# luisdamiano/sparseRGPs

Hardware: AMD Instinct MI355X
Metric: sparse-GP objective+gradient evals/sec at n=1e6, m=1024, d=8 (higher is better)
Workload: dtype f64; 1 GPU; C3: Titsias VI ELBO + gradient, n=1000000, m=1024, d=8, ard, P=10, knots fixed; n=1000000, m=1024, d=8, kernel=ard, parallelism=single

## Files before the change

### sparsergps_amd/csrc/k_mfma.hip

```cpp
#include <algorithm>
#include <vector>

#include "sgp_internal.h"
#include "sgp_probe.h"
#include "sgp_syrk_plan.h"

namespace {

constexpr int T128 = 128;
constexpr int BK = 16;
constexpr int SB = 144;
constexpr int SA = 17;
constexpr int SYRK_RGRP = 16;

__device__ __forceinline__ double wave_sum(double v) {
#pragma unroll
  for (int o = 32; o > 0; o >>= 1) v += __shfl_xor(v, o, 64);
  return v;
}

__device__ __forceinline__ int64_t xcd_remap(int64_t orig, int64_t nwg) {
  return sgp_plan::xcd_remap(orig, nwg);
}

__device__ __forceinline__ void load8(const double* __restrict__ g, double2 (&v)[4]) {
  const double2* p = reinterpret_cast<const double2*>(g);
#pragma unroll
  for (int q = 0; q < 4; ++q) v[q] = p[q];
}
__device__ __forceinline__ void store8(double* s, const double2 (&v)[4]) {
  double2* p = reinterpret_cast<double2*>(s);
#pragma unroll
  for (int q = 0; q < 4; ++q) p[q] = v[q];
}

__device__ __forceinline__ void syrk_group(int64_t gi, int nb, int wv, int& ta, int& tb, int& rs,
                                           int& cs, int& rp, int& cp) {
  const int64_t noff = (int64_t)nb * (nb - 1) / 2;
  if (gi < noff) {
    int a = (int)((sqrtf(8.0f * (float)gi + 1.0f) + 1.0f) * 0.5f);
    while ((int64_t)a * (a - 1) / 2 > gi) --a;
    while ((int64_t)(a + 1) * a / 2 <= gi) ++a;
    const int b = (int)(gi - (int64_t)a * (a - 1) / 2);
    ta = a; tb = b;
    const int wr = wv >> 1, wc = wv & 1;
    rs = wr; cs = 2 + wc;
    rp = 2 * a + wr; cp = 2 * b + wc;
    return;
  }
  const int g = (int)(gi - noff), G = (3 * nb + 3) / 4;
  const int te = G + g / 3, kind = g % 3;
  ta = g;
  tb = (te < nb) ? te : g;
  if (wv == 0) { rs = 0; cs = 0; rp = 2 * g; cp = 2 * g; }
  else if (wv == 1) { rs = 1; cs = 0; rp = 2 * g + 1; cp = 2 * g; }
  else if (wv == 2) { rs = 1; cs = 1; rp = 2 * g + 1; cp = 2 * g + 1; }
  else if (te < nb) {
    if (kind == 0) { rs = 2; cs = 2; rp = 2 * te; cp = 2 * te; }
    else if (kind == 1) { rs = 3; cs = 2; rp = 2 * te + 1; cp = 2 * te; }
    else { rs = 3; cs = 3; rp = 2 * te + 1; cp = 2 * te + 1; }
  } else {
    rs = cs = rp = cp = -1;
  }
}

struct SyrkTMap {
  signed char e[128];
  int S;
};

template <bool SPREAD = false, int PAT = 0, int NVMEM = 8, int NMFMA = 64>
__device__ __forceinline__ void mfma_interleave() {
#pragma unroll
  for (int i = 0; i < NMFMA; ++i) {
    __builtin_amdgcn_sched_group_barrier(0x008, 1, 0);
    if (i >= SGP_IL_VMEM0 && i < SGP_IL_VMEM0 + NVMEM)
      __builtin_amdgcn_sched_group_barrier(0x020, 1, 0);
    if (SPREAD ? (i & 1) == 0 : i < 32)
      __builtin_amdgcn_sched_group_barrier(0x100, 1, 0);
    constexpr int w0 = PAT == 2 ? NMFMA - 8 : PAT == 3 ? NMFMA / 2 : NMFMA - 16;
    if (PAT != 4 && i >= w0 && i < w0 + 8)
      __builtin_amdgcn_sched_group_barrier(0x200, 1, 0);
  }
}

template <int V, int WMODE, int TMODE, bool COMPACT = false>
__device__ __forceinline__ void syrk_dt_body(const double* __restrict__ K, int64_t mp,
                                             const double* __restrict__ w,
                                             const double* __restrict__ r,
                                             const double* __restrict__ tv, int t, int64_t rbeg,
                                             int nsteps, double (*Ka)[BK * SB], double (*ws)[BK],
                                             double (*rw)[BK], double& tacc, double& rrp,
                                             double* __restrict__ out) {
  constexpr int R0 = V, R1 = 7 - V, N0 = R0 + 1, N1 = R1 + 1;
  constexpr bool WITH_T = TMODE != 0;
  const int tid = threadIdx.x, lane = tid & 63;
  d4 acc0[N0], acc1[N1];
#pragma unroll
  for (int c = 0; c < N0; ++c) acc0[c] = d4{0.0, 0.0, 0.0, 0.0};
#pragma unroll
  for (int c = 0; c < N1; ++c) acc1[c] = d4{0.0, 0.0, 0.0, 0.0};
  const int lrow = tid >> 4, lc = tid & 15;
  const double2* gA = reinterpret_cast<const double2*>(K + (rbeg + lrow) * mp + t * (int64_t)T128) + lc;
  const int64_t gstep = BK * mp / 2;
  double2 v[4];
  double vw = 1.0, vsa = 1.0, vrr = 0.0, vr = 0.0;
  double t4[4] = {0.0, 0.0, 0.0, 0.0};
  const int tcol = tid & (T128 - 1), trow = tid >> 7;
#define SDT_GLOAD(step)                                                         \
  {                                                                             \
    const int64_t o_ = (int64_t)(step) * gstep;                                 \
    const int64_t rr_ = rbeg + (int64_t)(step) * BK + (tid & (BK - 1));        \
    _Pragma("unroll") for (int q = 0; q < 4; ++q) v[q] = gA[o_ + 16 * q];       \
    if constexpr (WMODE == 1) vw = w[rr_];                                      \
    if constexpr (WMODE == 2) vsa = w[rbeg + (int64_t)(step) * BK + lrow];      \
    if constexpr (WITH_T) {                                                     \
      vrr = r[rr_];                                                             \
      if constexpr (TMODE == 2) vr = tv[rr_];                                   \
    }                                                                           \
  }
#define SDT_SSTORE(buf, fold)                                                   \
  {                                                                             \
    double2* p_ = reinterpret_cast<double2*>(&Ka[buf][lrow * SB]) + lc;         \
    _Pragma("unroll") for (int q = 0; q < 4; ++q) {                             \
      double2 x_ = v[q];                                                        \
      if constexpr (WMODE == 2) { x_.x *= vsa; x_.y *= vsa; }                   \
      p_[16 * q] = x_;                                                          \
    }                                                                           \
    if constexpr (WMODE == 1) ws[buf][tid & (BK - 1)] = vw;                     \
    if constexpr (WITH_T) {                                                     \
      const double rw_ = TMODE == 2 ? vr : vw * vrr;                            \
      rw[buf][tid & (BK - 1)] = rw_;                                            \
      rrp = fma(rw_ * (fold), vrr, rrp);                                        \
    }                                                                           \
  }
  if (nsteps > 0) {
    SDT_GLOAD(0);
    SDT_SSTORE(0, 1.0);
  }
  __syncthreads();
  for (int step = 0; step < nsteps; ++step) {
    const int cur = step & 1;
    const bool more = step + 1 < nsteps;
    SDT_GLOAD(more ? step + 1 : step);
    const double* Kc = Ka[cur];
#pragma unroll
    for (int kk = 0; kk < 4; ++kk) {
      const int krow = kk * 4 + (lane >> 4);
      const double* row = Kc + krow * SB + (lane & 15);
      double a0 = row[R0 * 16], a1 = row[R1 * 16];
      if constexpr (WMODE == 1) {
        const double wk = ws[cur][krow];
        a0 *= wk;
        a1 *= wk;
      }
#pragma unroll
      for (int c = 0; c < N1; ++c) {
        const double b = row[c * 16];
        if (c < N0) acc0[c] = __builtin_amdgcn_mfma_f64_16x16x4f64(a0, b, acc0[c], 0, 0, 0);
        acc1[c] = __builtin_amdgcn_mfma_f64_16x16x4f64(a1, b, acc1[c], 0, 0, 0);
      }
    }
    if constexpr (WITH_T) {
#pragma unroll
      for (int k = 0; k < BK / 2; ++k) {
        const int q = trow + 2 * k;
        t4[k & 3] = fma(rw[cur][q], Kc[q * SB + tcol], t4[k & 3]);
      }
    }
    SDT_SSTORE(cur ^ 1, more ? 1.0 : 0.0);
    if constexpr (SGP_SDT_IL && WMODE != 1) mfma_interleave<false, 2, 4, 36>();
    __syncthreads();
  }
#undef SDT_GLOAD
#undef SDT_SSTORE
  tacc = (t4[0] + t4[1]) + (t4[2] + t4[3]);
#pragma unroll
  for (int c = 0; c < N1; ++c)
#pragma unroll
    for (int hh = 0; hh < 2; ++hh) {
      if (hh == 0 && c >= N0) continue;
      const int R = hh == 0 ? R0 : R1;
      const d4& a = hh == 0 ? acc0[c] : acc1[c];
      const int rp = 2 * t + R / 4, cp = 2 * t + c / 4;
      double* blk = out + (COMPACT ? (int64_t)(R / 4 + c / 4)
                                   : (int64_t)(rp * (rp + 1) / 2 + cp)) * 4096;
#pragma unroll
      for (int q = 0; q < 4; ++q)
        blk[((R % 4) * 16 + (lane >> 4) + 4 * q) * 64 + (c % 4) * 16 + (lane & 15)] = a[q];
    }
}

template <int WMODE, int TMODE>
__device__ __forceinline__ void syrk_dtile(const double* __restrict__ K, int64_t n_pad,
                                           int64_t mp, const double* __restrict__ w,
                                           const double* __restrict__ r,
                                           const double* __restrict__ tv, int t, int nb,
                                           int64_t sd, int64_t chunk, double (*Ka)[BK * SB],
                                           double (*ws)[BK], double (*rw)[BK],
                                           double* __restrict__ out,
                                           double* __restrict__ slab_t,
                                           double* __restrict__ slab_rr) {
  const int64_t rbeg = sd * chunk;
  int64_t rend = rbeg + chunk;
  if (rend > n_pad) rend = n_pad;
  const int nsteps = rend > rbeg ? (int)((rend - rbeg) / BK) : 0;
  double tacc = 0.0, rrp = 0.0;
  switch (threadIdx.x >> 6) {
    case 0: syrk_dt_body<0, WMODE, TMODE>(K, mp, w, r, tv, t, rbeg, nsteps, Ka, ws, rw, tacc, rrp, out); break;
    case 1: syrk_dt_body<1, WMODE, TMODE>(K, mp, w, r, tv, t, rbeg, nsteps, Ka, ws, rw, tacc, rrp, out); break;
    case 2: syrk_dt_body<2, WMODE, TMODE>(K, mp, w, r, tv, t, rbeg, nsteps, Ka, ws, rw, tacc, rrp, out); break;
    default: syrk_dt_body<3, WMODE, TMODE>(K, mp, w, r, tv, t, rbeg, nsteps, Ka, ws, rw, tacc, rrp, out); break;
  }
  if constexpr (TMODE != 0) {
    const int tid = threadIdx.x;
    double* tsh = &Ka[0][0];
    tsh[tid] = tacc;
    __syncthreads();
    if (tid < T128) slab_t[(sd * nb + t) * T128 + tid] = tsh[tid] + tsh[tid + T128];
    if (t == 0 && tid < 64) {
      double v = tid < BK ? rrp : 0.0;
#pragma unroll
      for (int o = 32; o > 0; o >>= 1) v += __shfl_xor(v, o, 64);
      if (tid == 0) slab_rr[sd] = v;
    }
  }
}

template <int TMODE, int WMODE, int TR = 2>
__global__ void __launch_bounds__(256, 2)
k_syrk_blk(const double* __restrict__ K, int64_t n_pad, int64_t mp, const double* __restrict__ w,
           const double* __restrict__ r, const double* __restrict__ tv,
           int64_t chunk, int ngroups, int nb, double* __restrict__ slab,
           double* __restrict__ slab_t, double* __restrict__ slab_rr, SyrkTMap tm,
           int64_t nwg_blk, int64_t chunk_d, double* __restrict__ slab_d) {
  __shared__ __attribute__((aligned(16))) double Ka[2][BK * SB];
  __shared__ __attribute__((aligned(16))) double Kb[2][BK * SB];
  __shared__ double ws[2][BK];
  __shared__ double rw[2][BK];

  if constexpr (TMODE == 0 || WMODE == 3) {
    if ((int64_t)blockIdx.x >= nwg_blk) {
      const int64_t loc = (int64_t)blockIdx.x - nwg_blk;
      const int t = (int)(loc % nb);
      const int64_t sd = loc / nb;
      syrk_dtile<WMODE == 3 ? 1 : WMODE, TMODE>(
          K, n_pad, mp, w, r, tv, t, nb, sd, chunk_d, Ka, ws, rw,
          slab_d + sd * ((int64_t)(2 * nb) * (2 * nb + 1) / 2) * 4096, slab_t, slab_rr);
      return;
    }
  }
  const int64_t nwg = nwg_blk;
  const int64_t wgid = xcd_remap(blockIdx.x, nwg);
  const int split = (int)(wgid / ngroups);
  const int64_t gi = wgid % ngroups;
// ... 87 lines not shown
  }
  __syncthreads();
  for (int step = 0; step < nsteps; ++step) {
    const int cur = step & 1;
    const bool more = step + 1 < nsteps;
    SYRKB_GLOAD(more ? step + 1 : step);
    if constexpr (WITH_T) __builtin_amdgcn_sched_barrier(0);
    const double* As = (ra ? Kb[cur] : Ka[cur]) + ro;
    const double* Bs = (ca_ ? Kb[cur] : Ka[cur]) + co;
    {
#pragma unroll
      for (int kk = 0; kk < 4; ++kk) {
        const int krow = kk * 4 + (lane >> 4);
        double af[4], bf[4];
#pragma unroll
        for (int f = 0; f < 4; ++f) {
          af[f] = As[krow * SB + f * 16 + (lane & 15)];
          bf[f] = Bs[krow * SB + f * 16 + (lane & 15)];
        }
        if constexpr (WMODE == 1) {
          const double wk = ws[cur][krow];
#pragma unroll
          for (int f = 0; f < 4; ++f) af[f] *= wk;
        }
#pragma unroll
        for (int fm = 0; fm < 4; ++fm)
#pragma unroll
          for (int fn = 0; fn < 4; ++fn)
            acc[fm][fn] = __builtin_amdgcn_mfma_f64_16x16x4f64(af[fm], bf[fn], acc[fm][fn], 0, 0, 0);
      }
    }
    SYRKB_SSTORE(cur ^ 1, more ? 1.0 : 0.0);
    mfma_interleave<false, SGP_SYRK_IL_PAT, WITH_T ? 0 : 8>();
    if constexpr (WITH_T) {
      const double* img = (t_inb ? Kb[cur] : Ka[cur]) + tcol;
      double a_[TR], b_[TR];
#pragma unroll
      for (int k = 0; k < TR; ++k) {
        const int q = trg + k * (BK / TR);
        a_[k] = rw[cur][q];
        b_[k] = img[q * SB];
      }
#pragma unroll
      for (int k = 0; k < TR; ++k) tacc4[k & 3] = fma(a_[k], b_[k], tacc4[k & 3]);
    }
    __syncthreads();
  }
#undef SYRKB_GLOAD
#undef SYRKB_SSTORE

  if constexpr (WITH_T) {
    __syncthreads();
    double* tsh = &Ka[0][0];
    if (t_on) tsh[tid] = (tacc4[0] + tacc4[1]) + (tacc4[2] + tacc4[3]);
    __syncthreads();
    if (t_on && tid < tW) {
      double v = 0.0;
      for (int g = 0; g < tng; ++g) v += tsh[tid + g * tW];
      slab_t[((int64_t)split * nb + tpan) * T128 + tcol] = v;
    }
  }
  if (dg == 0 && with_t && wv == 0) {
    double v = t_rr ? rrp : 0.0;
#pragma unroll
    for (int o = 32; o > 0; o >>= 1) v += __shfl_xor(v, o, 64);
    if (tid == 0) slab_rr[split] = v;
  }
  if (!active) return;
  const int64_t bid = (int64_t)rp * (rp + 1) / 2 + cp;
  const int64_t nblk = (int64_t)(2 * nb) * (2 * nb + 1) / 2;
  double* out = slab + ((int64_t)split * nblk + bid) * 4096;
#pragma unroll
  for (int fm = 0; fm < 4; ++fm)
#pragma unroll
    for (int fn = 0; fn < 4; ++fn)
#pragma unroll
      for (int q = 0; q < 4; ++q) {
        const int row = fm * 16 + (lane >> 4) + 4 * q;
        const int col = fn * 16 + (lane & 15);
        out[row * 64 + col] = acc[fm][fn][q];
      }
}

__device__ __forceinline__ void syrk_off_seg(const double* __restrict__ K, int64_t mp, int ta,
                                             int tb, int64_t rbeg, int nsteps,
                                             double (*Ka)[BK * SB], double (*Kb)[BK * SB],
                                             double* __restrict__ out) {
  const int tid = threadIdx.x, lane = tid & 63, wv = tid >> 6;
  d4 acc[4][4];
#pragma unroll
  for (int a = 0; a < 4; ++a)
#pragma unroll
    for (int b = 0; b < 4; ++b) acc[a][b] = d4{0.0, 0.0, 0.0, 0.0};
  const int lrow = tid >> 4, lc = tid & 15;
  const double2* gA = reinterpret_cast<const double2*>(K + (rbeg + lrow) * mp + ta * (int64_t)T128) + lc;
  const double2* gB = reinterpret_cast<const double2*>(K + (rbeg + lrow) * mp + tb * (int64_t)T128) + lc;
  const int64_t gstep = BK * mp / 2;
  double2 va0, va1, va2, va3, vb0, vb1, vb2, vb3;
  const int ro = (wv >> 1) * 64, co = (wv & 1) * 64;
#define SYRKO_GLOAD(step)                                                       \
  {                                                                             \
    const int64_t o_ = (int64_t)(step) * gstep;                                 \
    va0 = gA[o_]; va1 = gA[o_ + 16]; va2 = gA[o_ + 32]; va3 = gA[o_ + 48];      \
    vb0 = gB[o_]; vb1 = gB[o_ + 16]; vb2 = gB[o_ + 32]; vb3 = gB[o_ + 48];      \
  }
#define SYRKO_SSTORE(buf)                                                       \
  {                                                                             \
    double2* pa_ = reinterpret_cast<double2*>(&Ka[buf][lrow * SB]) + lc;        \
    double2* pb_ = reinterpret_cast<double2*>(&Kb[buf][lrow * SB]) + lc;        \
    pa_[0] = va0; pa_[16] = va1; pa_[32] = va2; pa_[48] = va3;                  \
    pb_[0] = vb0; pb_[16] = vb1; pb_[32] = vb2; pb_[48] = vb3;                  \
  }
  SYRKO_GLOAD(0);
  SYRKO_SSTORE(0);
  __syncthreads();
  for (int step = 0; step < nsteps; ++step) {
    const int cur = step & 1;
    const bool more = step + 1 < nsteps;
    SYRKO_GLOAD(more ? step + 1 : step);
    const double* As = Ka[cur] + ro;
    const double* Bs = Kb[cur] + co;
#pragma unroll
    for (int kk = 0; kk < 4; ++kk) {
      const int krow = kk * 4 + (lane >> 4);
      double af[4], bf[4];
#pragma unroll
      for (int f = 0; f < 4; ++f) {
        af[f] = As[krow * SB + f * 16 + (lane & 15)];
        bf[f] = Bs[krow * SB + f * 16 + (lane & 15)];
      }
#pragma unroll
      for (int fm = 0; fm < 4; ++fm)
#pragma unroll
        for (int fn = 0; fn < 4; ++fn)
          acc[fm][fn] = __builtin_amdgcn_mfma_f64_16x16x4f64(af[fm], bf[fn], acc[fm][fn], 0, 0, 0);
    }
    SYRKO_SSTORE(cur ^ 1);
    mfma_interleave<false, SGP_SYRK_IL_PAT, 8>();
    __syncthreads();
  }
#undef SYRKO_GLOAD
#undef SYRKO_SSTORE
  double* blk = out + (int64_t)wv * 4096;
#pragma unroll
  for (int fm = 0; fm < 4; ++fm)
#pragma unroll
    for (int fn = 0; fn < 4; ++fn)
#pragma unroll
      for (int q = 0; q < 4; ++q) {
        const int row = fm * 16 + (lane >> 4) + 4 * q;
        const int col = fn * 16 + (lane & 15);
        blk[row * 64 + col] = acc[fm][fn][q];
      }
}

__device__ __forceinline__ void syrk_diag_seg(const double* __restrict__ K, int64_t mp, int t,
                                              int64_t rbeg, int nsteps, double (*Ka)[BK * SB],
                                              double* __restrict__ out) {
  double tacc = 0.0, rrp = 0.0;
  switch (threadIdx.x >> 6) {
    case 0: syrk_dt_body<0, 0, 0, true>(K, mp, nullptr, nullptr, nullptr, t, rbeg, nsteps, Ka, nullptr, nullptr, tacc, rrp, out); break;
    case 1: syrk_dt_body<1, 0, 0, true>(K, mp, nullptr, nullptr, nullptr, t, rbeg, nsteps, Ka, nullptr, nullptr, tacc, rrp, out); break;
    case 2: syrk_dt_body<2, 0, 0, true>(K, mp, nullptr, nullptr, nullptr, t, rbeg, nsteps, Ka, nullptr, nullptr, tacc, rrp, out); break;
    default: syrk_dt_body<3, 0, 0, true>(K, mp, nullptr, nullptr, nullptr, t, rbeg, nsteps, Ka, nullptr, nullptr, tacc, rrp, out); break;
  }
}

__global__ void __launch_bounds__(256, 2)
k_syrk_bal(const double* __restrict__ K, int64_t mp, sgp_plan::SyrkBalPlan p,
           double* __restrict__ slab_o, double* __restrict__ slab_d) {
  __shared__ __attribute__((aligned(16))) double Ka[2][BK * SB];
  __shared__ __attribute__((aligned(16))) double Kb[2][BK * SB];
  const int wg = (int)blockIdx.x < p.M ? (int)xcd_remap(blockIdx.x, p.M) : (int)blockIdx.x;
  sgp_plan::SyrkSeg s0, s1;
  sgp_plan::syrk_bp_segments(p, wg, s0, s1);
  if (s0.kind == sgp_plan::SEG_OFF) {
    int ta, tb;
    sgp_plan::syrk_off_panels(s0.id, ta, tb);
    syrk_off_seg(K, mp, ta, tb, s0.step0 * BK, s0.nsteps, Ka, Kb,
                 slab_o + ((int64_t)s0.slab * p.noff + s0.id) * 4 * 4096);
  } else if (s0.kind == sgp_plan::SEG_DIAG) {
    syrk_diag_seg(K, mp, s0.id, s0.step0 * BK, s0.nsteps, Ka, slab_d + (int64_t)s0.slab * 3 * 4096);
  }
  if (s1.kind == sgp_plan::SEG_DIAG)
    syrk_diag_seg(K, mp, s1.id, s1.step0 * BK, s1.nsteps, Ka, slab_d + (int64_t)s1.slab * 3 * 4096);
}

__global__ void __launch_bounds__(256)
k_syrk_reduce_bal(const double* __restrict__ slab_o, const double* __restrict__ slab_d,
                  sgp_plan::SyrkBalPlan p, int64_t mp, double* __restrict__ red,
                  const double* __restrict__ rr_src, double* __restrict__ rr_dst, int packed) {
  const int64_t bid = blockIdx.y;
  const int e = blockIdx.x * 256 + threadIdx.x;
  if (rr_src && bid == 0 && e < 8) rr_dst[e] = e == 0 ? *rr_src : 0.0;
  int rp = (int)((sqrtf(8.0f * (float)bid + 1.0f) - 1.0f) * 0.5f);
  while ((int64_t)(rp + 1) * (rp + 2) / 2 <= bid) ++rp;
  while ((int64_t)rp * (rp + 1) / 2 > bid) --rp;
  const int cp = (int)(bid - (int64_t)rp * (rp + 1) / 2);
  const bool upper = rp == cp && (e / 64) / 16 < (e % 64) / 16;
  if (upper && !packed) return;
  if (!packed && rp == cp && (e / 64) < (e % 64)) return;
  const double* src;
  int64_t stride;
  int cnt;
  if (rp / 2 == cp / 2) {
    const int t = rp / 2;
    src = slab_d + ((int64_t)p.sfirst[t] * 3 + (rp & 1) + (cp & 1)) * 4096 + e;
    stride = 3 * 4096;
    cnt = p.sfirst[t + 1] - p.sfirst[t];
  } else {
    const int a = rp / 2, b = cp / 2, gi = a * (a - 1) / 2 + b;
    src = slab_o + ((int64_t)gi * 4 + (rp & 1) * 2 + (cp & 1)) * 4096 + e;
    stride = (int64_t)p.noff * 4 * 4096;
    cnt = p.B;
  }
  double v = 0.0;
  if (!upper)
    for (int s0 = 0; s0 < cnt; s0 += 16) {
      double a[16];
#pragma unroll
      for (int q = 0; q < 16; ++q) a[q] = s0 + q < cnt ? src[(int64_t)(s0 + q) * stride] : 0.0;
#pragma unroll
// ... 291 lines not shown
    double2* pb_ = reinterpret_cast<double2*>(&Kb[buf][lrow * SB]) + lc;        \
    pa_[0] = va0; pa_[16] = va1; pa_[32] = va2; pa_[48] = va3;                  \
    pb_[0] = vb0; pb_[16] = vb1; pb_[32] = vb2; pb_[48] = vb3;                  \
  }
  if (nsteps > 0) {
    TN_GLOAD(0);
    TN_SSTORE(0);
  }
  __syncthreads();
  for (int step = 0; step < nsteps; ++step) {
    const int cur = step & 1;
    if (step + 1 < nsteps) TN_GLOAD(step + 1);
    const double* As = Ka[cur];
    const double* Bs = Kb[cur];
#pragma unroll
    for (int kk = 0; kk < 4; ++kk) {
      const int krow = kk * 4 + (lane >> 4);
      double af[4], bf[4];
#pragma unroll
      for (int f = 0; f < 4; ++f) {
        af[f] = As[krow * SB + wr * 64 + f * 16 + (lane & 15)];
        bf[f] = Bs[krow * SB + wc * 64 + f * 16 + (lane & 15)];
      }
#pragma unroll
      for (int fm = 0; fm < 4; ++fm)
#pragma unroll
        for (int fn = 0; fn < 4; ++fn)
          acc[fm][fn] = __builtin_amdgcn_mfma_f64_16x16x4f64(af[fm], bf[fn], acc[fm][fn], 0, 0, 0);
    }
    if (step + 1 < nsteps) TN_SSTORE(cur ^ 1);
    __syncthreads();
  }
#undef TN_GLOAD
#undef TN_SSTORE
  double* out = slab + ((int64_t)split * ntile + tile) * (T128 * T128);
#pragma unroll
  for (int fm = 0; fm < 4; ++fm)
#pragma unroll
    for (int fn = 0; fn < 4; ++fn)
#pragma unroll
      for (int q = 0; q < 4; ++q) {
        const int row = wr * 64 + fm * 16 + (lane >> 4) + 4 * q;
        const int col = wc * 64 + fn * 16 + (lane & 15);
        out[row * T128 + col] = acc[fm][fn][q];
      }
}

__global__ void __launch_bounds__(256)
k_gemm_tn_reduce(const double* __restrict__ slab, int splits, int nta, int ntb,
                 double* __restrict__ C) {
  const int tile = blockIdx.y;
  const int e = blockIdx.x * 256 + threadIdx.x;
  const int ntile = nta * ntb;
  double s = 0.0;
  for (int sp = 0; sp < splits; ++sp) s += slab[((int64_t)sp * ntile + tile) * (T128 * T128) + e];
  const int ta = tile / ntb, tb = tile % ntb;
  const int64_t a = (int64_t)ta * T128 + e / T128, b = (int64_t)tb * T128 + e % T128;
  C[a * (int64_t)ntb * T128 + b] = s;
}

__global__ void __launch_bounds__(256)
k_syrk_reduce_t(const double* __restrict__ slab_t, const double* __restrict__ slab_rr,
                int splits, int nb, int64_t mp, double* __restrict__ red) {
  const int64_t a = (int64_t)blockIdx.x * 256 + threadIdx.x;
  if (a < mp) {
    const int ta = (int)(a / T128), col = (int)(a % T128);
    double s = 0.0;
    for (int sp = 0; sp < splits; ++sp) s += slab_t[((int64_t)sp * nb + ta) * T128 + col];
    red[mp * mp + a] = s;
  }
  if (blockIdx.x == 0 && threadIdx.x == 0) {
    double s = 0.0;
    for (int sp = 0; sp < splits; ++sp) s += slab_rr[sp];
    red[mp * mp + mp] = s;
  }
}

enum { EPI_GRAD = 0, EPI_ROWQUAD = 1 };

constexpr int CON_A_SZ = T128 * SA;
constexpr int CON_B_SZ = BK * SB;
constexpr int CON_LDS = 2 * (CON_A_SZ + CON_B_SZ);

enum { CON_FULL = 0, CON_TAIL = 1, CON_HEAD = 2 };
constexpr int64_t CON_SK_SLOT = 65 * 256;
struct ConSK {
  double* ws = nullptr;
  int dp = -1;
  unsigned* flags = nullptr;
  unsigned epoch = 0;
  int64_t slot = 0;
  int* status = nullptr;
};

__device__ __forceinline__ unsigned con_ldu_sc1(const unsigned* p) {
  return __hip_atomic_load(p, __ATOMIC_RELAXED, __HIP_MEMORY_SCOPE_AGENT);
}

template <int DT, int EPI, bool V2, bool KNOT, bool FROM_T, bool KU, bool T2, int SKM,
          bool VIF = false>
__device__ __forceinline__ void con_tile(
    const KernParams& kp, const double* __restrict__ K, const double* __restrict__ M,
    const double* __restrict__ X, int64_t ldx, int64_t n, int64_t n_pad,
    const double* __restrict__ U, int64_t ldu, int64_t m, int64_t mp, const ConArgs& ca,
    double* __restrict__ slab, int nrec, double* __restrict__ rowq, int64_t ti, int64_t tj,
    int64_t wgid, int kb, int ke, double* lds, double (*red)[SGP_MAXD + 5], double (*s_uk)[BK],
    const ConSK& sk, int part, int tid_in) {
  const double* __restrict__ r = ca.r;
  const double* __restrict__ uvec = ca.uvec;
  const double* __restrict__ cdiag = ca.cdiag;
  constexpr int A_SZ = CON_A_SZ, B_SZ = CON_B_SZ;
  const int64_t ntj = mp / T128;
  const int64_t nwg = (n_pad / T128) * ntj;
  const int64_t i0 = ti * T128, j0 = tj * T128;

  const int tid = tid_in, lane = tid & 63, wv = tid >> 6;
  const int wr = wv >> 1, wc = wv & 1;
  const bool with_u = KU && (uvec != nullptr) && (ca.alpha_in == nullptr);
  constexpr bool with_v = V2;
  constexpr bool NOCS = VIF && !KNOT;

  d4 acc[4][4];
#pragma unroll
  for (int a = 0; a < 4; ++a)
#pragma unroll
    for (int b = 0; b < 4; ++b) acc[a][b] = d4{0.0, 0.0, 0.0, 0.0};

  const int arow = tid >> 1, acol = (tid & 1) * 8;
  const double2* gA = reinterpret_cast<const double2*>(K + (i0 + arow) * mp + acol);
  const int bk = tid >> 4, bc = tid & 15;
  const double2* gB = reinterpret_cast<const double2*>(M + (int64_t)bk * mp + j0) + bc;
  const int64_t bstep = BK * mp / 2;
  double2 va0, va1, va2, va3, vb0, vb1, vb2, vb3;
  double ku = 0.0, vuk = 0.0;
  const double* __restrict__ uk_src = with_u ? uvec : M;

#define CON_GLOAD(step)                                                          \
  {                                                                              \
    const int64_t oa_ = (int64_t)(step) * (BK / 2), ob_ = (int64_t)(step) * bstep; \
    va0 = gA[oa_]; va1 = gA[oa_ + 1]; va2 = gA[oa_ + 2]; va3 = gA[oa_ + 3];      \
    vb0 = gB[ob_]; vb1 = gB[ob_ + 16]; vb2 = gB[ob_ + 32]; vb3 = gB[ob_ + 48];   \
    if constexpr (KU) vuk = uk_src[(int64_t)(step) * BK + (tid & (BK - 1))];     \
  }
#define CON_SSTORE(buf)                                                          \
  {                                                                              \
    double* As_ = lds + (buf) * (A_SZ + B_SZ);                                   \
    double* pa_ = &As_[arow * SA + acol];                                        \
    double2* pb_ = reinterpret_cast<double2*>(&As_[A_SZ + bk * SB]) + bc;        \
    pa_[0] = va0.x; pa_[1] = va0.y; pa_[2] = va1.x; pa_[3] = va1.y;              \
    pa_[4] = va2.x; pa_[5] = va2.y; pa_[6] = va3.x; pa_[7] = va3.y;              \
    pb_[0] = vb0; pb_[16] = vb1; pb_[32] = vb2; pb_[48] = vb3;                   \
    if constexpr (KU) s_uk[buf][tid & (BK - 1)] = vuk;    \
  }
#define CON_KU(buf)                                                              \
  {                                                                              \
    const double* u_ = &s_uk[buf][acol];                                         \
    ku = fma(va0.x, u_[0], ku); ku = fma(va0.y, u_[1], ku);                      \
    ku = fma(va1.x, u_[2], ku); ku = fma(va1.y, u_[3], ku);                      \
    ku = fma(va2.x, u_[4], ku); ku = fma(va2.y, u_[5], ku);                      \
    ku = fma(va3.x, u_[6], ku); ku = fma(va3.y, u_[7], ku);                      \
  }

  SGP_PROBE_CON_STAMP(0);
  if constexpr (FROM_T) {
#pragma unroll
    for (int fm = 0; fm < 4; ++fm)
#pragma unroll
      for (int fn = 0; fn < 4; ++fn)
#pragma unroll
        for (int q = 0; q < 4; ++q)
          acc[fm][fn][q] = ca.tin[(i0 + wr * 64 + fm * 16 + (lane >> 4) + 4 * q) * mp + j0 +
                                  wc * 64 + fn * 16 + (lane & 15)];
  } else {
  CON_GLOAD(kb);
  CON_SSTORE(0);
  __syncthreads();
  for (int step = kb; step < ke; ++step) {
    const int cur = (step - kb) & 1;
    if constexpr (KU) CON_KU(cur);
    CON_GLOAD(step + 1 < ke ? step + 1 : step);
    const double* As = lds + cur * (A_SZ + B_SZ);
    const double* Bs = As + A_SZ;
#pragma unroll
    for (int kk = 0; kk < 4; ++kk) {
      const int kx = kk * 4 + (lane >> 4);
      double af[4], bf[4];
#pragma unroll
      for (int f = 0; f < 4; ++f) {
        af[f] = As[(wr * 64 + f * 16 + (lane & 15)) * SA + kx];
        bf[f] = Bs[kx * SB + wc * 64 + f * 16 + (lane & 15)];
      }
#pragma unroll
      for (int fm = 0; fm < 4; ++fm)
#pragma unroll
        for (int fn = 0; fn < 4; ++fn)
          acc[fm][fn] = __builtin_amdgcn_mfma_f64_16x16x4f64(af[fm], bf[fn], acc[fm][fn], 0, 0, 0);
    }
    CON_SSTORE(cur ^ 1);
    mfma_interleave<SGP_CON_IL_SPREAD, SGP_CON_IL_PAT>();
    __syncthreads();
  }
  }
#undef CON_GLOAD
#undef CON_SSTORE
#undef CON_KU

  if constexpr (SKM == CON_TAIL) {
    double* w = sk.ws + sk.slot * CON_SK_SLOT;
#pragma unroll
    for (int fm = 0; fm < 4; ++fm)
#pragma unroll
      for (int fn = 0; fn < 4; ++fn)
#pragma unroll
        for (int q = 0; q < 4; ++q)
          __hip_atomic_store(&w[((fm * 4 + fn) * 4 + q) * 256 + tid], acc[fm][fn][q],
                             __ATOMIC_RELAXED, __HIP_MEMORY_SCOPE_AGENT);
    __hip_atomic_store(&w[64 * 256 + tid], ku, __ATOMIC_RELAXED, __HIP_MEMORY_SCOPE_AGENT);
    asm volatile("s_waitcnt vmcnt(0)" ::: "memory");
    __syncthreads();
    if (tid == 0)
      __hip_atomic_store(&sk.flags[sk.slot], sk.epoch, __ATOMIC_RELAXED, __HIP_MEMORY_SCOPE_AGENT);
    return;
  }
  if (SKM == CON_HEAD && part == CON_HEAD) {
    if (tid == 0) {
      unsigned it = 0;
      while (con_ldu_sc1(&sk.flags[sk.slot]) != sk.epoch) {
        if (++it >= (1u << 22)) {
          atomicExch(sk.status, -1);
          break;
        }
        __builtin_amdgcn_s_sleep(1);
      }
    }
    __syncthreads();
    const double* w = sk.ws + sk.slot * CON_SK_SLOT;
#pragma unroll
    for (int fm = 0; fm < 4; ++fm) {
      double t[4][4];
#pragma unroll
      for (int fn = 0; fn < 4; ++fn)
#pragma unroll
        for (int q = 0; q < 4; ++q)
          t[fn][q] = __hip_atomic_load(&w[((fm * 4 + fn) * 4 + q) * 256 + tid], __ATOMIC_RELAXED,
                                       __HIP_MEMORY_SCOPE_AGENT);
#pragma unroll
      for (int fn = 0; fn < 4; ++fn)
#pragma unroll
        for (int q = 0; q < 4; ++q) acc[fm][fn][q] += t[fn][q];
      __builtin_amdgcn_sched_barrier(0);
    }
    ku += __hip_atomic_load(&w[64 * 256 + tid], __ATOMIC_RELAXED, __HIP_MEMORY_SCOPE_AGENT);
  }

  SGP_PROBE_CON_STAMP(1);
// ... 236 lines not shown
        const bool cok = 8 * ch + cc < d;
        double E = 0.0;
#pragma unroll
        for (int fn = 0; fn < 4; ++fn) {
          if constexpr (NOCS) {
#pragma unroll
            for (int q = 0; q < 4; ++q) {
              const int jl = wc * 64 + fn * 16 + (lane >> 4) + 4 * q;
              const double u = cok ? s_us[jl * sus + cc] : 0.0;
              const double pv = P[fn][q];
              E += (cp >= 8) ? pv : -2.0 * (u * pv);
            }
          } else {
          double C = Cc[fn];
          C += __shfl_xor(C, 16, 64);
          C += __shfl_xor(C, 32, 64);
          if (ch == 0 && (lane >> 4) == 0) e_sig += C;
#pragma unroll
          for (int q = 0; q < 4; ++q) {
            const int jl = wc * 64 + fn * 16 + (lane >> 4) + 4 * q;
            const double Cq = __shfl(C, (lane >> 4) + 4 * q, 64);
            const double u = cok ? s_us[jl * sus + cc] : 0.0;
            const double pv = P[fn][q];
            E += (cp >= 8) ? pv : u * fma(u, Cq, -2.0 * pv);
            if constexpr (KNOT) {
              if (cp < 8) s_kn[(wr * T128 + jl) * 8 + cc] = pv - u * Cq;
            }
          }
          }
        }
        E += __shfl_xor(E, 8, 64);
        E += __shfl_xor(E, 16, 64);
        E += __shfl_xor(E, 32, 64);
        if (ard) {
          if (lane < 8 && 8 * ch + lane < d) red[wv][1 + 8 * ch + lane] = E;
        } else {
          double t = E;
          t += __shfl_xor(t, 1, 64);
          t += __shfl_xor(t, 2, 64);
          t += __shfl_xor(t, 4, 64);
          e_sq += t;
        }
        if constexpr (KNOT) {
          __syncthreads();
          for (int e = tid; e < T128 * 8; e += 256) {
            const int col = e >> 3, c = e & 7, cg = 8 * ch + c;
            if (cg < d)
              ca.knot_slab[(ti * mp + j0 + col) * d + cg] =
                  s_kn[col * 8 + c] + s_kn[(T128 + col) * 8 + c];
          }
        }
      }
#undef CON_XSTAGE
    }

    SGP_PROBE_CON_STAMP(6);
    double v = 0.0;
    if constexpr (!NOCS) v = wave_sum(e_sig);
    if (lane == 0) red[wv][0] = v;
    if (!ard && lane == 0) red[wv][1] = e_sq * rl2s;
    v = 0.0;
    if constexpr (!VIF) v = wave_sum(a2);
    if (lane == 0) {
      red[wv][1 + L] = 0.0;
      red[wv][2 + L] = 0.0;
      red[wv][3 + L] = 0.0;
      red[wv][4 + L] = v;
    }
    __syncthreads();
    if (tid < nrec)
      slab[tid * nwg + wgid] = red[0][tid] + red[1][tid] + red[2][tid] + red[3][tid];
    SGP_PROBE_CON_STAMP(2);
  }
  if constexpr (SGP_CON_EPI_PRIO > 0) __builtin_amdgcn_s_setprio(0);
}

template <int DT, int EPI, bool V2 = false, bool KNOT = false, bool FROM_T = false, bool KU = true,
          bool T2 = false, bool VIF = false>
__global__ void __launch_bounds__(256, 2)
k_contract(KernParams kp, const double* __restrict__ K, const double* __restrict__ M,
           const double* __restrict__ X, int64_t ldx, int64_t n, int64_t n_pad,
           const double* __restrict__ U, int64_t ldu, int64_t m, int64_t mp, ConArgs ca,
           double* __restrict__ slab, int nrec, double* __restrict__ rowq) {
  __shared__ __attribute__((aligned(16))) double lds[CON_LDS];
  __shared__ double red[4][SGP_MAXD + 5];
  __shared__ double s_uk[2][BK];
  const int64_t ntj = mp / T128;
  const int64_t nwg = (n_pad / T128) * ntj;
  const int64_t wgid = xcd_remap(blockIdx.x, nwg);
  con_tile<DT, EPI, V2, KNOT, FROM_T, KU, T2, 0, VIF>(
      kp, K, M, X, ldx, n, n_pad, U, ldu, m, mp, ca, slab, nrec, rowq, wgid / ntj, wgid % ntj,
      wgid, 0, (int)(mp / BK), lds, red, s_uk, ConSK{}, CON_FULL, (int)threadIdx.x);
}

template <int DT, bool KNOT, bool VIF = false>
__global__ void __launch_bounds__(256, 2)
k_contract_sk(KernParams kp, const double* __restrict__ K, const double* __restrict__ M,
              const double* __restrict__ X, int64_t ldx, int64_t n, int64_t n_pad,
              const double* __restrict__ U, int64_t ldu, int64_t m, int64_t mp, ConArgs ca,
              double* __restrict__ slab, int nrec, ConSK sk) {
  __shared__ __attribute__((aligned(16))) double lds[CON_LDS];
  __shared__ double red[4][SGP_MAXD + 5];
  __shared__ double s_uk[2][BK];
  const int64_t ntj = mp / T128;
  const int64_t ntiles = (n_pad / T128) * ntj;
  const int S = (int)(mp / BK);
  const int64_t G = gridDim.x, v = xcd_remap(blockIdx.x, G);
  const int64_t dp_rounds = (sk.dp >= 0 && sk.dp < ntiles / G) ? sk.dp : ntiles / G - 1;
  const int64_t t0 = dp_rounds * G;
  const int64_t Usk = (ntiles - t0) * S;
  const int64_t u1 = Usk * (v + 1) / G;
  int64_t u = Usk * v / G;
  if (u % S != 0) {
    const int64_t tile = t0 + u / S;
    const int kb = (int)(u % S);
    ConSK p = sk;
    p.slot = v;
    con_tile<DT, EPI_GRAD, false, KNOT, false, !VIF, false, CON_TAIL, VIF>(
        kp, K, M, X, ldx, n, n_pad, U, ldu, m, mp, ca, slab, nrec, nullptr, tile / ntj,
        tile % ntj, tile, kb, S, lds, red, s_uk, p, CON_TAIL, (int)threadIdx.x);
    u += S - kb;
    __syncthreads();
  }
  int64_t r = 0;
  for (;;) {
    int64_t tile;
    int ke;
    if (r < dp_rounds) {
      tile = r * G + v;
      ke = S;
      ++r;
    } else if (u < u1) {
      tile = t0 + u / S;
      ke = (int)((u1 - u) < (int64_t)S ? (u1 - u) : S);
      u += ke;
    } else {
      break;
    }
    ConSK p = sk;
    p.slot = v + 1;
    int tid;
    asm volatile("v_mov_b32 %0, %1" : "=v"(tid) : "v"((int)threadIdx.x));
    con_tile<DT, EPI_GRAD, false, KNOT, false, !VIF, false, CON_HEAD, VIF>(
        kp, K, M, X, ldx, n, n_pad, U, ldu, m, mp, ca, slab, nrec, nullptr, tile / ntj,
        tile % ntj, tile, 0, ke, lds, red, s_uk, p, ke < S ? CON_HEAD : CON_FULL, tid);
    __syncthreads();
  }
}

__global__ void __launch_bounds__(256)
k_knot_reduce1(const double* __restrict__ slab, int64_t ntiles, int64_t ncol,
               double* __restrict__ part) {
  const int64_t col = (int64_t)blockIdx.x * 256 + threadIdx.x;
  const int64_t r = blockIdx.y, G = gridDim.y;
  if (col >= ncol) return;
  double s0 = 0.0, s1 = 0.0, s2 = 0.0, s3 = 0.0;
  int64_t t = r;
  for (; t + 3 * G < ntiles; t += 4 * G) {
    s0 += slab[t * ncol + col];
    s1 += slab[(t + G) * ncol + col];
    s2 += slab[(t + 2 * G) * ncol + col];
    s3 += slab[(t + 3 * G) * ncol + col];
  }
  for (; t < ntiles; t += G) s0 += slab[t * ncol + col];
  part[r * ncol + col] = (s0 + s1) + (s2 + s3);
}

// ... 852 lines not shown
```

### sparsergps_amd/csrc/sgp_probe.h

```cpp
#pragma once

#if (defined(SGP_CON_TRACE) || defined(SGP_CON_NO_EPILOGUE) || defined(SGP_GJ_TRACE) ||       \
     defined(SGP_IL_VMEM0) || defined(SGP_CON_IL_PAT) || defined(SGP_SYRK_IL_PAT) ||          \
     defined(SGP_CON_IL_SPREAD) || defined(SGP_CON_SHMEM) ||                                  \
     defined(SGP_SYRK_BAL) || defined(SGP_SYRK_WB) || defined(SGP_SYRK_WB_SLOTS) ||           \
     defined(SGP_SDT_IL) || defined(SGP_S256_IL) ||                  \
     defined(SGP_SDT_W) || defined(SGP_SDT_WW) || defined(SGP_SDT_WT) ||                      \
     defined(SGP_SYRK_W3) || defined(SGP_CON_ROWQ_KU) ||                                      \
     defined(SGP_LAP_RS_CFG) || defined(SGP_GJ_MM_UNROLL) || defined(SGP_VI_BUILD_NO_T) ||        \
     defined(SGP_GJ_STEPS) || defined(SGP_GJ_GMAX) || defined(SGP_CHAIN_US_STEP) ||         \
     defined(SGP_CHAIN_US_FIX) || defined(SGP_HOST_PROBE) || defined(SGP_BUILD_OCC_T2) ||      \
     defined(SGP_CON_EPI_PRIO) || defined(SGP_CON_PROBE_NO_EPI_MFMA) ||                       \
     defined(SGP_CON_PROBE_NO_KDMA)) &&      \
    !defined(SGP_PROBE_BUILD)
#error "timing probes and experiment knobs are for variant builds only (SGP_PROBE_BUILD)"
#endif

#ifndef SGP_CON_EPI_PRIO
#define SGP_CON_EPI_PRIO 0
#endif
#ifndef SGP_BUILD_OCC_T2
#define SGP_BUILD_OCC_T2 4
#endif
#ifndef SGP_IL_VMEM0
#define SGP_IL_VMEM0 0
#endif
#ifndef SGP_CON_IL_PAT
#define SGP_CON_IL_PAT 2
#endif
#ifndef SGP_SYRK_IL_PAT
#define SGP_SYRK_IL_PAT 0
#endif
#ifndef SGP_CON_IL_SPREAD
#define SGP_CON_IL_SPREAD false
#endif
#ifndef SGP_CON_SHMEM
#define SGP_CON_SHMEM 0
#endif
#ifndef SGP_SYRK_BAL
#define SGP_SYRK_BAL 1
#endif
#ifndef SGP_SYRK_WB
#define SGP_SYRK_WB 1
#endif
#ifndef SGP_SYRK_WB_SLOTS
#define SGP_SYRK_WB_SLOTS 512
#endif
#ifndef SGP_SDT_IL
#define SGP_SDT_IL 1
#endif
#ifndef SGP_SDT_W
#define SGP_SDT_W 38
#endif
#ifndef SGP_SDT_WW
#define SGP_SDT_WW 2
#endif
#ifndef SGP_SDT_WT
#define SGP_SDT_WT 6
#endif
#ifndef SGP_SYRK_W3
#define SGP_SYRK_W3 1
#endif
#ifndef SGP_CON_ROWQ_KU
#define SGP_CON_ROWQ_KU 0
#endif
#ifndef SGP_LAP_RS_CFG
#define SGP_LAP_RS_CFG 0
#endif
#ifndef SGP_GJ_MM_UNROLL
#define SGP_GJ_MM_UNROLL 16
#endif
#ifndef SGP_S256_IL
#define SGP_S256_IL 0
#endif
#ifndef SGP_GJ_STEPS
#define SGP_GJ_STEPS 0
#endif
#ifndef SGP_GJ_GMAX
#define SGP_GJ_GMAX 128
#endif
#ifndef SGP_CHAIN_US_STEP
#define SGP_CHAIN_US_STEP 60.0
#endif
#ifndef SGP_CHAIN_US_FIX
#define SGP_CHAIN_US_FIX 250.0
#endif
#ifndef SGP_VI_BUILD_NO_T
#define SGP_VI_BUILD_NO_T 0
#endif

#ifdef SGP_CON_TRACE
#define SGP_PROBE_CON_STAMP(k_)        \
  do {                                 \
    if (tid == 0) SGP_CON_TRACE(k_);   \
  } while (0)
#else
#define SGP_PROBE_CON_STAMP(k_) \
  do {                          \
  } while (0)
#endif

#ifdef SGP_CON_NO_EPILOGUE
#define SGP_PROBE_CON_SKIP_EPILOGUE()                                                   \
  if constexpr (EPI == EPI_GRAD) {                                                      \
    double v_ = 0.0;                                                                    \
    _Pragma("unroll") for (int fm_ = 0; fm_ < 4; ++fm_)                                 \
      _Pragma("unroll") for (int fn_ = 0; fn_ < 4; ++fn_)                               \
        v_ += acc[fm_][fn_][0] + acc[fm_][fn_][3];                                      \
    if (v_ == 1234.5) slab[tid] = v_;                                                   \
    return;                                                                             \
  }
#else
#define SGP_PROBE_CON_SKIP_EPILOGUE()
#endif

#ifdef SGP_GJ_TRACE
#define SGP_PROBE_GJ_DECL() const bool gj_tr_ = (i == k + 1) && (j == k + 1) && threadIdx.x == 0
#define SGP_PROBE_GJ_STAMP(p_)          \
  do {                                  \
    if (gj_tr_) SGP_GJ_TRACE(k, p_);    \
// ... 10 lines not shown
```

Before: 21.29 evals/s.

## Replace double-buffered LDS with four-slot half-step ring in SYRK and contraction kernels

Adds a four-slot LDS ring of half-K-step (BK/2) sub-tiles to the diagonal SYRK, off-diagonal SYRK and VI contraction kernels. Global loads run three sub-steps ahead, and LDS fragment reads for the next sub-step are issued before the barrier, so each synchronisation covers half a tile and MFMA work overlaps memory traffic with explicit sched_group_barrier interleaving. Both paths are enabled by default through new macros. The cost is more register pressure and more barriers per K-step, and the contraction kernel needs a larger LDS allocation with a padded A layout, which may reduce occupancy.

```diff
diff --git a/sparsergps_amd/csrc/k_mfma.hip b/sparsergps_amd/csrc/k_mfma.hip
--- a/sparsergps_amd/csrc/k_mfma.hip
+++ b/sparsergps_amd/csrc/k_mfma.hip
@@ -81,6 +81,21 @@
     constexpr int w0 = PAT == 2 ? NMFMA - 8 : PAT == 3 ? NMFMA / 2 : NMFMA - 16;
     if (PAT != 4 && i >= w0 && i < w0 + 8)
       __builtin_amdgcn_sched_group_barrier(0x200, 1, 0);
+  }
+}
+
+constexpr int SYRK_RING_HS = (BK / 2) * SB;
+template <int NRD, int NWR, int NMFMA = 32, int NVMEM = 4>
+__device__ __forceinline__ void ring_interleave() {
+#pragma unroll
+  for (int i = 0; i < NMFMA; ++i) {
+    __builtin_amdgcn_sched_group_barrier(0x008, 1, 0);
+    if (i < NVMEM) __builtin_amdgcn_sched_group_barrier(0x020, 1, 0);
+    if (i < NRD) __builtin_amdgcn_sched_group_barrier(0x100, 1, 0);
+    if (i >= NMFMA / 2 && i < NMFMA / 2 + NRD)
+      __builtin_amdgcn_sched_group_barrier(0x100, 1, 0);
+    constexpr int w0 = NMFMA - 4 - NWR;
+    if (i >= w0 && i < w0 + NWR) __builtin_amdgcn_sched_group_barrier(0x200, 1, 0);
   }
 }
 
@@ -134,6 +149,77 @@
       rrp = fma(rw_ * (fold), vrr, rrp);                                        \
     }                                                                           \
   }
+  if constexpr (COMPACT && WMODE == 0 && TMODE == 0 && SGP_SYRK_RING != 0) {
+    double* Rk = &Ka[0][0];
+    const int rrow = tid >> 5, rc = tid & 31;
+    const double2* rA = reinterpret_cast<const double2*>(K + (rbeg + rrow) * mp + t * (int64_t)T128) + rc;
+    const int64_t rsub = (BK / 2) * mp / 2;
+    const int nsub = 2 * nsteps;
+    double2 p0, p1, q0, q1;
+    double s0[N1];
+    int fo[4][2];
+#pragma unroll
+    for (int b = 0; b < 4; ++b)
+#pragma unroll
+      for (int sl = 0; sl < 2; ++sl) {
+        fo[b][sl] = b * SYRK_RING_HS + (sl * 4 + (lane >> 4)) * SB + (lane & 15);
+        asm volatile("" : "+v"(fo[b][sl]));
+      }
+#define RING_LOAD(sub_, A0, A1)                                                 \
+  {                                                                             \
+    const int s_ = (sub_) < nsub ? (sub_) : nsub - 1;      \
+    A0 = rA[(int64_t)s_ * rsub]; A1 = rA[(int64_t)s_ * rsub + 32];              \
+  }
+#define RING_STORE(buf_, A0, A1)                                                \
+  {                                                                             \
+    double2* p_ = reinterpret_cast<double2*>(Rk + (buf_) * SYRK_RING_HS + rrow * SB) + rc; \
+    p_[0] = A0; p_[32] = A1;                                                    \
+  }
+#define RING_READ(buf_, sl_, F)                                                 \
+  _Pragma("unroll") for (int c = 0; c < N1; ++c) F[c] = Rk[fo[buf_][sl_] + c * 16];
+#define RING_MFMA(F)                                                            \
+  _Pragma("unroll") for (int c = 0; c < N1; ++c) {                              \
+    if (c < N0) acc0[c] = __builtin_amdgcn_mfma_f64_16x16x4f64(F[R0], F[c], acc0[c], 0, 0, 0); \
+    acc1[c] = __builtin_amdgcn_mfma_f64_16x16x4f64(F[R1], F[c], acc1[c], 0, 0, 0); \
+  }
+#define RING_SUB(j_, R_, L0, L1, S0, S1)                                        \
+  {                                                                             \
+    RING_LOAD((j_) + 3, L0, L1);                                                \
+    double s1_[N1], n0_[N1];                                                    \
+    RING_READ(R_, 1, s1_);                                                      \
+    RING_MFMA(s0);                                                              \
+    RING_READ(((R_) + 1) & 3, 0, n0_);                                          \
+    RING_MFMA(s1_);                                                             \
+    RING_STORE(((R_) + 2) & 3, S0, S1);                                         \
+    ring_interleave<4, 2, 18, 2>();                                             \
+    __syncthreads();                                                            \
+    __builtin_amdgcn_sched_barrier(0);                                          \
+    _Pragma("unroll") for (int c = 0; c < N1; ++c) s0[c] = n0_[c];              \
+  }
+    RING_LOAD(0, p0, p1);
+    RING_LOAD(1, q0, q1);
+    RING_STORE(0, p0, p1);
+    RING_STORE(1, q0, q1);
+    RING_LOAD(2, p0, p1);
+    __syncthreads();
+    RING_READ(0, 0, s0);
+    int j = 0;
+    for (; j + 4 <= nsub; j += 4) {
+      RING_SUB(j, 0, q0, q1, p0, p1);
+      RING_SUB(j + 1, 1, p0, p1, q0, q1);
+      RING_SUB(j + 2, 2, q0, q1, p0, p1);
+      RING_SUB(j + 3, 3, p0, p1, q0, q1);
+    }
+    if (j < nsub) {
+      RING_SUB(j, 0, q0, q1, p0, p1);
+      RING_SUB(j + 1, 1, p0, p1, q0, q1);
+    }
+#undef RING_SUB
+#undef RING_MFMA
+#undef RING_READ
+#undef RING_STORE
+#undef RING_LOAD
+  } else {
   if (nsteps > 0) {
     SDT_GLOAD(0);
     SDT_SSTORE(0, 1.0);
@@ -171,6 +257,7 @@
     SDT_SSTORE(cur ^ 1, more ? 1.0 : 0.0);
     if constexpr (SGP_SDT_IL && WMODE != 1) mfma_interleave<false, 2, 4, 36>();
     __syncthreads();
+  }
   }
 #undef SDT_GLOAD
 #undef SDT_SSTORE
@@ -424,6 +511,7 @@
       }
 }
 
+
 __device__ __forceinline__ void syrk_off_seg(const double* __restrict__ K, int64_t mp, int ta,
                                              int tb, int64_t rbeg, int nsteps,
                                              double (*Ka)[BK * SB], double (*Kb)[BK * SB],
@@ -453,6 +541,85 @@
     pa_[0] = va0; pa_[16] = va1; pa_[32] = va2; pa_[48] = va3;                  \
     pb_[0] = vb0; pb_[16] = vb1; pb_[32] = vb2; pb_[48] = vb3;                  \
   }
+  if constexpr (SGP_SYRK_RING) {
+    constexpr int HS = SYRK_RING_HS;
+    double* Ra = &Ka[0][0];
+    double* Rb = &Kb[0][0];
+    const int rrow = tid >> 5, rc = tid & 31;
+    const double2* rA = reinterpret_cast<const double2*>(K + (rbeg + rrow) * mp + ta * (int64_t)T128) + rc;
+    const double2* rB = reinterpret_cast<const double2*>(K + (rbeg + rrow) * mp + tb * (int64_t)T128) + rc;
+    const int64_t rsub = (BK / 2) * mp / 2;
+    const int nsub = 2 * nsteps;
+    double2 pa0, pa1, pb0, pb1;
+    double2 qa0, qa1, qb0, qb1;
+    double a0[4], b0[4];
+#define RING_LOAD(sub_, A0, A1, B0, B1)                                         \
+  {                                                                             \
+    const int s_ = (sub_) < nsub ? (sub_) : nsub - 1;      \
+    const int64_t o_ = (int64_t)s_ * rsub;                                      \
+    A0 = rA[o_]; A1 = rA[o_ + 32]; B0 = rB[o_]; B1 = rB[o_ + 32];               \
+  }
+#define RING_STORE(buf_, A0, A1, B0, B1)                                        \
+  {                                                                             \
+    double2* pa_ = reinterpret_cast<double2*>(Ra + (buf_) * HS + rrow * SB) + rc; \
+    double2* pb_ = reinterpret_cast<double2*>(Rb + (buf_) * HS + rrow * SB) + rc; \
+    pa_[0] = A0; pa_[32] = A1; pb_[0] = B0; pb_[32] = B1;                       \
+  }
+    int fo[4][2];
+#pragma unroll
+    for (int b = 0; b < 4; ++b)
+#pragma unroll
+      for (int sl = 0; sl < 2; ++sl) {
+        fo[b][sl] = b * HS + (sl * 4 + (lane >> 4)) * SB + (lane & 15);
+        asm volatile("" : "+v"(fo[b][sl]));
+      }
+#define RING_READ(buf_, sl_, AF, BF)                                            \
+  _Pragma("unroll") for (int f = 0; f < 4; ++f) {                               \
+    AF[f] = Ra[fo[buf_][sl_] + ro + f * 16];                                    \
+    BF[f] = Rb[fo[buf_][sl_] + co + f * 16];                                    \
+  }
+#define RING_MFMA(AF, BF)                                                       \
+  _Pragma("unroll") for (int fm = 0; fm < 4; ++fm)                              \
+    _Pragma("unroll") for (int fn = 0; fn < 4; ++fn)                            \
+      acc[fm][fn] = __builtin_amdgcn_mfma_f64_16x16x4f64(AF[fm], BF[fn], acc[fm][fn], 0, 0, 0);
+#define RING_SUB(j_, R_, L0, L1, L2, L3, S0, S1, S2, S3)                        \
+  {                                                                             \
+    RING_LOAD((j_) + 3, L0, L1, L2, L3);                                        \
+    double a1_[4], b1_[4], na_[4], nb_[4];                                      \
+    RING_READ(R_, 1, a1_, b1_);                                                 \
+    RING_MFMA(a0, b0);                                                          \
+    RING_READ(((R_) + 1) & 3, 0, na_, nb_);                                     \
+    RING_MFMA(a1_, b1_);                                                        \
+    RING_STORE(((R_) + 2) & 3, S0, S1, S2, S3);                                 \
+    ring_interleave<4, 4>();                                                    \
+    __syncthreads();                                                            \
+    __builtin_amdgcn_sched_barrier(0);                                          \
+    _Pragma("unroll") for (int f = 0; f < 4; ++f) { a0[f] = na_[f]; b0[f] = nb_[f]; } \
+  }
+    RING_LOAD(0, pa0, pa1, pb0, pb1);
+    RING_LOAD(1, qa0, qa1, qb0, qb1);
+    RING_STORE(0, pa0, pa1, pb0, pb1);
+    RING_STORE(1, qa0, qa1, qb0, qb1);
+    RING_LOAD(2, pa0, pa1, pb0, pb1);
+    __syncthreads();
+    RING_READ(0, 0, a0, b0);
+    int j = 0;
+    for (; j + 4 <= nsub; j += 4) {
+      RING_SUB(j, 0, qa0, qa1, qb0, qb1, pa0, pa1, pb0, pb1);
+      RING_SUB(j + 1, 1, pa0, pa1, pb0, pb1, qa0, qa1, qb0, qb1);
+      RING_SUB(j + 2, 2, qa0, qa1, qb0, qb1, pa0, pa1, pb0, pb1);
+      RING_SUB(j + 3, 3, pa0, pa1, pb0, pb1, qa0, qa1, qb0, qb1);
+    }
+    if (j < nsub) {
+      RING_SUB(j, 0, qa0, qa1, qb0, qb1, pa0, pa1, pb0, pb1);
+      RING_SUB(j + 1, 1, pa0, pa1, pb0, pb1, qa0, qa1, qb0, qb1);
+    }
+#undef RING_SUB
+#undef RING_MFMA
+#undef RING_READ
+#undef RING_STORE
+#undef RING_LOAD
+  } else {
   SYRKO_GLOAD(0);
   SYRKO_SSTORE(0);
   __syncthreads();
@@ -480,6 +647,7 @@
     SYRKO_SSTORE(cur ^ 1);
     mfma_interleave<false, SGP_SYRK_IL_PAT, 8>();
     __syncthreads();
+  }
   }
 #undef SYRKO_GLOAD
 #undef SYRKO_SSTORE
@@ -937,6 +1105,17 @@
 constexpr int CON_B_SZ = BK * SB;
 constexpr int CON_LDS = 2 * (CON_A_SZ + CON_B_SZ);
 
+constexpr int SA8 = 9;
+constexpr int CON_RING_A = T128 * SA8;
+constexpr int CON_RING_SUB = CON_RING_A + (BK / 2) * SB;
+constexpr int CON_LDS_RING = 4 * CON_RING_SUB;
+constexpr int CON_RING_NRD = 4;
+constexpr int CON_RING_NWR = 4;
+template <bool FROM_T, bool KU, int SKM, bool VIF>
+constexpr bool con_ring() {
+  return SGP_CON_RING && VIF && !KU && !FROM_T && SKM == 0;
+}
+
 enum { CON_FULL = 0, CON_TAIL = 1, CON_HEAD = 2 };
 constexpr int64_t CON_SK_SLOT = 65 * 256;
 struct ConSK {
@@ -974,6 +1153,7 @@
   const bool with_u = KU && (uvec != nullptr) && (ca.alpha_in == nullptr);
   constexpr bool with_v = V2;
   constexpr bool NOCS = VIF && !KNOT;
+  constexpr bool RING = con_ring<FROM_T, KU, SKM, VIF>();
 
   d4 acc[4][4];
 #pragma unroll
@@ -1026,6 +1206,72 @@
         for (int q = 0; q < 4; ++q)
           acc[fm][fn][q] = ca.tin[(i0 + wr * 64 + fm * 16 + (lane >> 4) + 4 * q) * mp + j0 +
                                   wc * 64 + fn * 16 + (lane & 15)];
+  } else if constexpr (RING) {
+    const int rrow = (tid & 15) + 16 * (tid >> 5), rh = ((tid >> 4) & 1) * 4;
+    const double2* rA = reinterpret_cast<const double2*>(K + (i0 + rrow) * mp + rh);
+    const int rbk = tid >> 5, rbc = tid & 31;
+    const double2* rB = reinterpret_cast<const double2*>(M + (int64_t)rbk * mp + j0) + rbc;
+    const int64_t rbstep = (BK / 2) * mp / 2;
+    double2 pa0, pa1, pb0, pb1;
+    double2 qa0, qa1, qb0, qb1;
+    double a0[4], b0[4];
+#define RING_LOAD(sub_, A0, A1, B0, B1)                                          \
+  {                                                                              \
+    const int64_t oa_ = (int64_t)(sub_) * (BK / 4), ob_ = (int64_t)(sub_) * rbstep; \
+    A0 = rA[oa_]; A1 = rA[oa_ + 1]; B0 = rB[ob_]; B1 = rB[ob_ + 32];             \
+  }
+#define RING_STORE(buf_, A0, A1, B0, B1)                                         \
+  {                                                                              \
+    double* As_ = lds + (buf_) * CON_RING_SUB;                                   \
+    double* pa_ = &As_[rrow * SA8 + rh];                                         \
+    double2* pb_ = reinterpret_cast<double2*>(&As_[CON_RING_A + rbk * SB]) + rbc; \
+    pa_[0] = A0.x; pa_[1] = A0.y; pa_[2] = A1.x; pa_[3] = A1.y;                  \
+    pb_[0] = B0; pb_[32] = B1;                                                   \
+  }
+#define RING_READ(buf_, sl_, AF, BF)                                             \
+  _Pragma("unroll") for (int f = 0; f < 4; ++f) {                                \
+    const double* As_ = lds + (buf_) * CON_RING_SUB;                             \
+    const int kx_ = (sl_) * 4 + (lane >> 4);                                     \
+    AF[f] = As_[(wr * 64 + f * 16 + (lane & 15)) * SA8 + kx_];                   \
+    BF[f] = As_[CON_RING_A + kx_ * SB + wc * 64 + f * 16 + (lane & 15)];         \
+  }
+#define RING_MFMA(AF, BF)                                                        \
+  _Pragma("unroll") for (int fm = 0; fm < 4; ++fm)                               \
+    _Pragma("unroll") for (int fn = 0; fn < 4; ++fn)                             \
+      acc[fm][fn] = __builtin_amdgcn_mfma_f64_16x16x4f64(AF[fm], BF[fn], acc[fm][fn], 0, 0, 0);
+#define RING_SUB(j_, R_, L0, L1, L2, L3, S0, S1, S2, S3)                         \
+  {                                                                              \
+    RING_LOAD((j_) + 3 < sub_end ? (j_) + 3 : sub_end - 1, L0, L1, L2, L3);      \
+    double a1_[4], b1_[4], na_[4], nb_[4];                                       \
+    RING_READ(R_, 1, a1_, b1_);                                                  \
+    RING_MFMA(a0, b0);                                                           \
+    RING_READ(((R_) + 1) & 3, 0, na_, nb_);                                      \
+    RING_MFMA(a1_, b1_);                                                         \
+    RING_STORE(((R_) + 2) & 3, S0, S1, S2, S3);                                  \
+    ring_interleave<CON_RING_NRD, CON_RING_NWR>();                               \
+    __syncthreads();                                                             \
+    __builtin_amdgcn_sched_barrier(0);                                           \
+    _Pragma("unroll") for (int f = 0; f < 4; ++f) { a0[f] = na_[f]; b0[f] = nb_[f]; } \
+  }
+    const int sub_beg = 2 * kb, sub_end = 2 * ke;
+    RING_LOAD(sub_beg, pa0, pa1, pb0, pb1);
+    RING_LOAD(sub_beg + 1, qa0, qa1, qb0, qb1);
+    RING_STORE(0, pa0, pa1, pb0, pb1);
+    RING_STORE(1, qa0, qa1, qb0, qb1);
+    RING_LOAD(sub_beg + 2, pa0, pa1, pb0, pb1);
+    __syncthreads();
+    RING_READ(0, 0, a0, b0);
+    for (int j = sub_beg; j < sub_end; j += 4) {
+      RING_SUB(j, 0, qa0, qa1, qb0, qb1, pa0, pa1, pb0, pb1);
+      RING_SUB(j + 1, 1, pa0, pa1, pb0, pb1, qa0, qa1, qb0, qb1);
+      RING_SUB(j + 2, 2, qa0, qa1, qb0, qb1, pa0, pa1, pb0, pb1);
+      RING_SUB(j + 3, 3, pa0, pa1, pb0, pb1, qa0, qa1, qb0, qb1);
+    }
+#undef RING_SUB
+#undef RING_MFMA
+#undef RING_READ
+#undef RING_STORE
+#undef RING_LOAD
   } else {
   CON_GLOAD(kb);
   CON_SSTORE(0);
@@ -1428,7 +1674,8 @@
            const double* __restrict__ X, int64_t ldx, int64_t n, int64_t n_pad,
            const double* __restrict__ U, int64_t ldu, int64_t m, int64_t mp, ConArgs ca,
            double* __restrict__ slab, int nrec, double* __restrict__ rowq) {
-  __shared__ __attribute__((aligned(16))) double lds[CON_LDS];
+  __shared__ __attribute__((aligned(16))) double
+      lds[con_ring<FROM_T, KU, 0, VIF>() ? CON_LDS_RING : CON_LDS];
   __shared__ double red[4][SGP_MAXD + 5];
   __shared__ double s_uk[2][BK];
   const int64_t ntj = mp / T128;
diff --git a/sparsergps_amd/csrc/sgp_probe.h b/sparsergps_amd/csrc/sgp_probe.h
--- a/sparsergps_amd/csrc/sgp_probe.h
+++ b/sparsergps_amd/csrc/sgp_probe.h
@@ -11,7 +11,8 @@
      defined(SGP_GJ_STEPS) || defined(SGP_GJ_GMAX) || defined(SGP_CHAIN_US_STEP) ||         \
      defined(SGP_CHAIN_US_FIX) || defined(SGP_HOST_PROBE) || defined(SGP_BUILD_OCC_T2) ||      \
      defined(SGP_CON_EPI_PRIO) || defined(SGP_CON_PROBE_NO_EPI_MFMA) ||                       \
-     defined(SGP_CON_PROBE_NO_KDMA)) &&      \
+     defined(SGP_CON_PROBE_NO_KDMA) || defined(SGP_CON_RING) ||       \
+     defined(SGP_SYRK_RING)) &&      \
     !defined(SGP_PROBE_BUILD)
 #error "timing probes and experiment knobs are for variant builds only (SGP_PROBE_BUILD)"
 #endif
@@ -36,6 +37,12 @@
 #endif
 #ifndef SGP_CON_SHMEM
 #define SGP_CON_SHMEM 0
+#endif
+#ifndef SGP_CON_RING
+#define SGP_CON_RING 1
+#endif
+#ifndef SGP_SYRK_RING
+#define SGP_SYRK_RING 1
 #endif
 #ifndef SGP_SYRK_BAL
 #define SGP_SYRK_BAL 1
```

Result: faster. 22.02 evals/s, median of 6 (+3.5%).
